# maxgillett/tinysplat

Measured on AMD Instinct MI355X. Metric: Gaussians*pixels/s fwd+bwd, higher is better.
Workload: dtype f32; 1 GPU; 1000000 random Gaussians, SH degree 3, 1920x1080, fwd+bwd (RGB), BASELINE configs[2]; max_per_tile=614, parallelism=single GPU, tile_lists=16x16 (gsplat's) (auto), gaussian_order=as generated (i.i.d.)

## Files before the change

tinysplat_amd/csrc/binning.hip:

```cpp
#include <hip/hip_runtime.h>

#include "../../include/tinysplat_hip.h"
#include "host_util.h"
#include "pack.h"
#include "row_spans.h"
#include "splat_math.h"

namespace {

constexpr int kThreads = 256;
constexpr int kScanItems = 4;
constexpr int kScanBlock = kThreads * kScanItems;

__device__ __forceinline__ int wave_inclusive_scan(int v) {
    const int lane = threadIdx.x & 63;
#pragma unroll
    for (int d = 1; d < 64; d <<= 1) {
        const int u = __shfl_up(v, d, 64);
        if (lane >= d) v += u;
    }
    return v;
}

template <int WAVES = 4>
// ... 989 lines not shown
    } else {
        walk([&](int t, int len, int i) {
            const int at = atomicAdd(&c.cursor[t >> kCoarseShift], len);
            for (int q = 0; q < len; ++q) dst[at + q] = i | (((t + q) & (kCoarseTiles - 1)) << kCoarseIdBits);
        });
    }
}

#ifndef TS_RUN_AHEAD
#define TS_RUN_AHEAD 20
#endif
constexpr int kRunItems = TS_RUN_AHEAD;
constexpr int kRunPass = kFineThreads * kRunItems;
#ifndef TS_RUNS_IN_FLIGHT
#define TS_RUNS_IN_FLIGHT 8
#endif
constexpr int kRunAhead = TS_RUNS_IN_FLIGHT;
__global__ __launch_bounds__(kFineThreads) void bin_scatter_fine_runs_kernel(
    int num_tiles, int groups, int chunks, const int* __restrict__ counts, const int* __restrict__ starts,
    int* __restrict__ tile_start, int* __restrict__ tile_bins, int* __restrict__ group_max,
    const int* __restrict__ scratch, int* __restrict__ bucket_ids) {
    extern __shared__ unsigned int buf[];
    const int my_count = (int)threadIdx.x < chunks ? counts[(size_t)threadIdx.x * groups + blockIdx.x] : 0;
    const int my_start = (int)threadIdx.x < chunks ? starts[(size_t)threadIdx.x * groups + blockIdx.x] : 0;
    const int begin = tile_start[min(num_tiles, (int)(blockIdx.x << kCoarseShift))];
    if (tile_start[num_tiles + 1] != 0) return;
    __shared__ FineGroup sh;
    __shared__ int roff[kBinMaxChunks + 1], rsrc[kBinMaxChunks];
    constexpr int kWaves = kFineThreads / 64;
    const int tid = threadIdx.x, lane = tid & 63, wave = tid >> 6;
    const int t0 = blockIdx.x << kCoarseShift, t1 = min(num_tiles, t0 + kCoarseTiles);
    if (tid < kCoarseTiles) {
        sh.hist[tid] = 0;
        sh.cursor[tid] = 0;
    }
    int total;
    {
        const int c = my_count;
        const int inc = block_inclusive_scan<kWaves>(c, &total);
        if (tid < chunks) {
            roff[tid] = inc - c;
            rsrc[tid] = my_start;
        }
        if (tid == 0) roff[chunks] = total;
    }
    __syncthreads();
    auto for_runs = [&](int c0, int m, auto op) {
#pragma unroll 1
        for (int b0 = wave; b0 < chunks; b0 += kWaves * kRunAhead) {
            int len[kRunAhead], src[kRunAhead], dst[kRunAhead];
            unsigned int v[kRunAhead];
#pragma unroll
            for (int u = 0; u < kRunAhead; ++u) {
                const int b = b0 + u * kWaves;
                len[u] = src[u] = dst[u] = 0;
                if (b < chunks) {
                    const int o = roff[b], c = roff[b + 1] - o;
                    const int lo = max(0, c0 - o) + lane;
                    len[u] = min(c, c0 + m - o) - lo;
                    src[u] = rsrc[b] + lo;
                    dst[u] = o - c0 + lo;
                }
            }
#pragma unroll
            for (int u = 0; u < kRunAhead; ++u)
                if (len[u] > 0) v[u] = (unsigned int)scratch[src[u]];
#pragma unroll
            for (int u = 0; u < kRunAhead; ++u)
                if (len[u] > 0) op(dst[u], v[u]);
#pragma unroll
            for (int u = 0; u < kRunAhead; ++u)
                for (int j = 64; j < len[u]; j += 64) op(dst[u] + j, (unsigned int)scratch[src[u] + j]);
        }
    };
    const GroupLists lists{t0, t1, begin, tile_start, tile_bins, group_max};
    const bool counted = total > kRunPass || total == 0;
    if (counted) {
        for_runs(0, total, [&](int, unsigned int w) { atomicAdd(&sh.hist[w >> kCoarseIdBits], 1); });
        publish_counted(sh, lists);
    }
    for (int c0 = 0; c0 < total; c0 += kRunPass) {
        const int m = min(kRunPass, total - c0);
        for_runs(c0, m, [&](int k, unsigned int w) { buf[k] = w; });
        __syncthreads();
        place_pass<kRunItems>(sh, buf, m, [&](int k) { return buf[k]; }, !counted, lists, bucket_ids);
    }
}

struct ListStats {
    const int* group_max;
    const int* guard;
    int* longest_out;
    int groups;
};
__device__ __forceinline__ void store_longest(const ListStats& st) {
    __shared__ int longest;
    if (threadIdx.x == 0) longest = 0;
    __syncthreads();
    int m = 0;
    for (int g = threadIdx.x; g < st.groups; g += kThreads) m = max(m, st.group_max[g]);
#pragma unroll
    for (int d = 32; d >= 1; d >>= 1) m = max(m, __shfl_xor(m, d, 64));
    if ((threadIdx.x & 63) == 0) atomicMax(&longest, m);
    __syncthreads();
    if (threadIdx.x == 0 && *st.guard == 0) *st.longest_out = longest;
}

constexpr int kSortCap = 4096;

#include "sort_network.h"

struct IdKeyArray {
    volatile int* ids;
    const float* depths;
};

__device__ __forceinline__ void cmpswap(IdKeyArray a, int i, int j) {
    const int x = a.ids[i], y = a.ids[j];
    if (make_key(a.depths, x) > make_key(a.depths, y)) { a.ids[i] = y; a.ids[j] = x; }
}

template <typename Ptr>
__device__ __forceinline__ void bitonic_network(Ptr a, int n) {
    int lg = 0;
    while ((1 << lg) < n) ++lg;
    const int half = (1 << lg) >> 1;
    for (int lk = 1; lk <= lg; ++lk) {
        const int k = 1 << lk, hk = k >> 1;
        for (int p = threadIdx.x; p < half; p += kThreads) {
            const int base = (p >> (lk - 1)) << lk, off = p & (hk - 1);
            const int i = base + off, j = base + k - 1 - off;
            if (j < n) cmpswap(a, i, j);
        }
        __syncthreads();
        for (int ld = lk - 2; ld >= 0; --ld) {
            const int d = 1 << ld;
            for (int p = threadIdx.x; p < half; p += kThreads) {
                const int i = ((p >> ld) << (ld + 1)) | (p & (d - 1)), j = i + d;
                if (j < n) cmpswap(a, i, j);
            }
            __syncthreads();
        }
    }
}

template <int E>
__device__ __forceinline__ void sort_tile_regs(const int* g, const float* __restrict__ depths,
                                               int* out, int n, unsigned long long* lds) {
    const int t = threadIdx.x;
    unsigned long long k[E];
#pragma unroll
    for (int e = 0; e < E; ++e) {
        const int i = t * E + e;
        k[e] = i < n ? make_key(depths, g[i]) : ~0ull;
    }
    __syncthreads();
    bitonic_regs<E, kThreads>(k, t, min(pow2_at_least(n), kThreads * E), lds);
#pragma unroll
    for (int e = 0; e < E; ++e) {
        const int i = t * E + e;
        if (i < n) out[i] = (int)(unsigned int)k[e];
    }
}

__device__ __forceinline__ void sort_bucket_block(const int* g, const float* __restrict__ depths,
                                                  int* out, int n, unsigned long long* lds) {
    if (n <= kThreads) sort_tile_regs<1>(g, depths, out, n, lds);
    else if (n <= 2 * kThreads) sort_tile_regs<2>(g, depths, out, n, lds);
    else if (n <= 4 * kThreads) sort_tile_regs<4>(g, depths, out, n, lds);
    else if (n <= 8 * kThreads) sort_tile_regs<8>(g, depths, out, n, lds);
    else sort_tile_regs<16>(g, depths, out, n, lds);
}

constexpr int kMaxSub = 512;
constexpr int kSubTarget = 96;
constexpr int kLargeLdsU64 = kSortCap + 2048;

__device__ __forceinline__ void sort_tile_sample(const int* __restrict__ g,
                                                 const float* __restrict__ depths,
                                                 int* __restrict__ out, int n,
                                                 unsigned long long* lds) {
    unsigned long long* scratch = lds;
    unsigned long long* smp = lds + kSortCap;
    int* start = reinterpret_cast<int*>(lds + kSortCap + 1024);
    int* cursor = start + (kMaxSub + 1);
    int* big = cursor + kMaxSub;
    __shared__ int nbig;
    const int t = threadIdx.x, lane = t & 63, wave = t >> 6;
    const int ns = n > 8192 ? 1024 : 256;
    int nb = n / kSubTarget;
    nb = nb < 2 ? 2 : (nb > kMaxSub ? kMaxSub : nb);

    if (ns == 1024) {
        unsigned long long k[4];
#pragma unroll
        for (int e = 0; e < 4; ++e)
            k[e] = make_key(depths, g[(int)(((long long)(t * 4 + e) * n) >> 10)]);
        bitonic_regs<4, kThreads>(k, t, 1024, scratch);
#pragma unroll
        for (int e = 0; e < 4; ++e) smp[t * 4 + e] = k[e];
    } else {
        unsigned long long k[1];
        k[0] = make_key(depths, g[(int)(((long long)t * n) >> 8)]);
        bitonic_regs<1, kThreads>(k, t, 256, scratch);
        smp[t] = k[0];
    }
    for (int b = t; b < nb; b += kThreads) cursor[b] = 0;
    if (t == 0) nbig = 0;
    __syncthreads();

    auto sub_of = [&](unsigned long long key) {
        int lo = 0, hi = nb - 1;
        while (lo < hi) {
            const int mid = (lo + hi) >> 1;
            if (smp[((mid + 1) * ns) / nb] <= key) lo = mid + 1; else hi = mid;
        }
        return lo;
    };
    for (int i = t; i < n; i += kThreads) atomicAdd(&cursor[sub_of(make_key(depths, g[i]))], 1);
    __syncthreads();
    {
        const int c0 = (2 * t < nb) ? cursor[2 * t] : 0, c1 = (2 * t + 1 < nb) ? cursor[2 * t + 1] : 0;
        int total;
        const int inc = block_inclusive_scan(c0 + c1, &total);
        const int ex = inc - (c0 + c1);
        if (2 * t < nb) start[2 * t] = ex;
        if (2 * t + 1 < nb) start[2 * t + 1] = ex + c0;
        if (t == 0) start[nb] = n;
    }
    __syncthreads();
    for (int b = t; b < nb; b += kThreads) cursor[b] = start[b];
    __syncthreads();
    for (int i = t; i < n; i += kThreads) {
        const int id = g[i];
        out[atomicAdd(&cursor[sub_of(make_key(depths, id))], 1)] = id;
    }
    __threadfence_block();
    __syncthreads();
    for (int b = wave; b < nb; b += kThreads / 64) {
        const int s0 = start[b], m = start[b + 1] - s0;
        if (m <= 1) continue;
        if (m <= 256) {
            unsigned long long k[4];
#pragma unroll
            for (int e = 0; e < 4; ++e) {
                const int i = lane * 4 + e;
                k[e] = i < m ? make_key(depths, out[s0 + i]) : ~0ull;
            }
            bitonic_regs<4, 64>(k, lane, min(pow2_at_least(m), 256), nullptr);
#pragma unroll
            for (int e = 0; e < 4; ++e) {
                const int i = lane * 4 + e;
                if (i < m) out[s0 + i] = (int)(unsigned int)k[e];
            }
        } else if (lane == 0) {
            big[atomicAdd(&nbig, 1)] = b;
        }
    }
    __syncthreads();
    const int nbg = nbig;
    for (int q = 0; q < nbg; ++q) {
        const int b = big[q];
        const int s0 = start[b], m = start[b + 1] - s0;
        __syncthreads();
        if (m <= kSortCap) {
            sort_bucket_block(out + s0, depths, out + s0, m, scratch);
        } else {
            IdKeyArray a{out + s0, depths};
            bitonic_network(a, m);
        }
        __syncthreads();
    }
}

__global__ __launch_bounds__(kThreads) void sort_tiles_small_kernel(
    int num_tiles, const int* __restrict__ tile_bins, const float* __restrict__ depths,
    const int* __restrict__ bucket_ids, int* __restrict__ ids_sorted, int* __restrict__ large_count,
    int* __restrict__ large_list, const ListStats stats) {
    if (stats.group_max && blockIdx.x == 0) store_longest(stats);
    const int lane = threadIdx.x & 63;
    const int tile = blockIdx.x * (kThreads / 64) + (threadIdx.x >> 6);
    if (tile >= num_tiles) return;
    const int2 range = reinterpret_cast<const int2*>(tile_bins)[tile];
    const int n = range.y - range.x;
    if (n <= 0) return;
    if (n > kWaveSortMax) {
        if (n > kSortCap && lane == 0) large_list[atomicAdd(large_count, 1)] = tile;
        return;
    }
    const int* g = bucket_ids + range.x;
    int* out = ids_sorted + range.x;
    if (n <= 64) sort_tile_wave<1>(g, depths, out, n, lane);
    else if (n <= 128) sort_tile_wave<2>(g, depths, out, n, lane);
    else if (n <= 256) sort_tile_wave<4>(g, depths, out, n, lane);
    else if (n <= 512) sort_tile_wave<8>(g, depths, out, n, lane);
    else sort_tile_wave<16>(g, depths, out, n, lane);
}

__global__ __launch_bounds__(kThreads) void sort_tiles_mid_kernel(
    const int* __restrict__ tile_bins, const float* __restrict__ depths,
    const int* __restrict__ bucket_ids, int* __restrict__ ids_sorted, int* __restrict__ large_count,
    int* __restrict__ large_list) {
    __shared__ unsigned long long lk[kSortCap / 2];
    const int2 range = reinterpret_cast<const int2*>(tile_bins)[blockIdx.x];
    const int n = range.y - range.x;
    if (n > kSortCap && large_count && threadIdx.x == 0) large_list[atomicAdd(large_count, 1)] = blockIdx.x;
    if (n <= kWaveSortMax || n > kSortCap) return;
    sort_bucket_block(bucket_ids + range.x, depths, ids_sorted + range.x, n, lk);
}

__global__ __launch_bounds__(kThreads) void sort_tiles_large_kernel(
    const int* __restrict__ tile_bins, const float* __restrict__ depths,
    const int* __restrict__ bucket_ids, int* __restrict__ ids_sorted,
    const int* __restrict__ large_count, const int* __restrict__ large_list) {
    __shared__ unsigned long long lds_large[kLargeLdsU64];
    const int count = *large_count;
    for (int q = blockIdx.x; q < count; q += gridDim.x) {
        const int2 range = reinterpret_cast<const int2*>(tile_bins)[large_list[q]];
        const int n = range.y - range.x;
        if (n <= kSortCap) continue;
        __syncthreads();
        sort_tile_sample(bucket_ids + range.x, depths, ids_sorted + range.x, n, lds_large);
    }
}

__global__ __launch_bounds__(kThreads) void sort_tiles_above_kernel(
    const int* __restrict__ tile_bins, const float* __restrict__ depths,
    const int* __restrict__ bucket_ids, int* __restrict__ ids_sorted, const ListStats stats) {
    __shared__ unsigned long long lds_u64[kLargeLdsU64 > kSortCap / 2 ? kLargeLdsU64 : kSortCap / 2];
    if (stats.group_max && blockIdx.x == 0) store_longest(stats);
    const int2 range = reinterpret_cast<const int2*>(tile_bins)[blockIdx.x];
    const int n = range.y - range.x;
    if (n <= kWaveSortMax) return;
    if (n <= kSortCap) sort_bucket_block(bucket_ids + range.x, depths, ids_sorted + range.x, n, lds_u64);
    else sort_tile_sample(bucket_ids + range.x, depths, ids_sorted + range.x, n, lds_u64);
}

__global__ __launch_bounds__(kThreads) void pack_splats_kernel(int n, const ts::PackArgs a,
                                                              const float* __restrict__ colors) {
    const int i = blockIdx.x * kThreads + threadIdx.x;
    if (i >= n) return;
    if (a.radii[i] <= 0) return;
    float c0, c1, c2, c3 = 0.0f;
    if (a.channels == 4 && a.depths == nullptr) {
        const float4 c = reinterpret_cast<const float4*>(colors)[i];
        c0 = c.x; c1 = c.y; c2 = c.z; c3 = c.w;
    } else {
        c0 = colors[3 * i]; c1 = colors[3 * i + 1]; c2 = colors[3 * i + 2];
        if (a.channels == 4) c3 = a.depths[i];
    }
    ts::pack_one(a, i, c0, c1, c2, c3);
}

template <typename... Params, typename... Args>
void launch_with_lds(void (*kernel)(Params...), dim3 grid, dim3 block, size_t lds, hipStream_t s, Args... args) {
    if (lds > 64 * 1024)
        (void)hipFuncSetAttribute(reinterpret_cast<const void*>(kernel), hipFuncAttributeMaxDynamicSharedMemorySize,
                                  (int)lds);
    hipLaunchKernelGGL(kernel, grid, block, lds, s, args...);
}

}

extern "C" {

int32_t ts_num_tiles(const ts_camera* cam) {
    if (!cam) return 0;
    const int tbx = cam->wide_tiles ? (cam->tile_bounds_x + 1) / 2 : cam->tile_bounds_x;
    return cam->tile_rows * tbx;
}

int64_t ts_scan_ws_ints(int32_t n) {
    return n <= 0 ? 1 : (int64_t)((n + kScanBlock - 1) / kScanBlock);
}

int ts_scan_tiles(int32_t n, const int32_t* num_tiles_hit, int32_t* cum_tiles_hit,
                  int32_t* scan_ws, int32_t* total_out, void* stream) {
    if (n < 0) return TS_E_BADARG;
    if (n == 0) return 0;
    if (!num_tiles_hit || !cum_tiles_hit || !scan_ws) return TS_E_BADARG;
    hipStream_t s = (hipStream_t)stream;
    const int nb = (n + kScanBlock - 1) / kScanBlock;
    hipLaunchKernelGGL(scan_local_kernel, dim3(nb), dim3(kThreads), 0, s, n, num_tiles_hit,
                       cum_tiles_hit, scan_ws, total_out);
    if (nb > 1)
        hipLaunchKernelGGL(scan_add_kernel, dim3(nb), dim3(kThreads), 0, s, n, cum_tiles_hit, scan_ws,
                           total_out);
    return launch_status();
}

int64_t ts_bin_ws_ints(int32_t n, int32_t num_tiles) { return bin_geometry(n, num_tiles).spare + 1; }

int ts_bin_count(int32_t n, const float* xys, const int32_t* radii, const float* splats,
                 const ts_camera* cam, int32_t* bin_ws, void* stream) {
    if (n < 0 || !cam || !bin_ws) return TS_E_BADARG;
    const int nt = ts_num_tiles(cam);
    if (nt <= 0) return 0;
    if (n > 0 && (!xys || !radii)) return TS_E_BADARG;
    const BinGeometry g = bin_geometry(n, nt);
    const int window = bin_window_tiles(n, nt);
// ... 261 lines not shown
```

tinysplat_amd/csrc/raster.hip:

```cpp
#include <hip/hip_runtime.h>

#include <type_traits>

#include "../../include/tinysplat_hip.h"
#include "host_util.h"
#include "raster_survivors.h"
#include "splat_math.h"

namespace {
#include "sort_network.h"

#ifndef TS_FWD_MIN_WAVES_RGB
#define TS_FWD_MIN_WAVES_RGB 5
#endif
#ifndef TS_FWD_MIN_WAVES_RGBD
#define TS_FWD_MIN_WAVES_RGBD 5
#endif
#ifndef TS_BWD_MIN_WAVES_16
#define TS_BWD_MIN_WAVES_16 5
#endif

#ifndef TS_ABLATE
#define TS_ABLATE 0
#endif
// ... 298 lines not shown
        "v_fma_f32 %2, -%1, %5, %5\n\t"
        "v_sub_f32_e32 %3, %5, %2\n\t"
        "v_cmp_nge_f32_e32 vcc, %16, %2\n\t"
        "v_cndmask_b32_e32 %4, 0, %3, vcc\n\t"
        "v_fmac_f32_e32 %6, %11, %4\n\t"
        "v_fmac_f32_e32 %7, %12, %4\n\t"
        "v_cndmask_b32_e64 %5, -|%5|, %2, vcc\n\t"
        "v_fmac_f32_e32 %8, %13, %4\n\t"
        "v_cmp_lt_f32_e32 vcc, 0, %4\n\t"
        "v_cndmask_b32_e32 %9, %9, %14, vcc"
        : "=&v"(a), "=&v"(ae), "=&v"(nT), "=&v"(d), "=&v"(vis), "+v"(T), "+v"(a0), "+v"(a1), "+v"(a2), "+v"(fidx)
        : "v"(sgl), "v"(c0), "v"(c1), "v"(c2), "v"(idx), "s"(ts::kAlphaMin), "s"(ts::kTEps)
        : "vcc");
    return vis;
}
__device__ __forceinline__ float fwd_update(float ae, float& T, int& fidx, int idx, float& a0, float& a1, float& a2,
                                            float c0, float c1, float c2) {
    float nT, d, vis;
    asm("v_fma_f32 %0, -%8, %3, %3\n\t"
        "v_sub_f32_e32 %1, %3, %0\n\t"
        "v_cmp_nge_f32_e32 vcc, %13, %0\n\t"
        "v_cndmask_b32_e32 %2, 0, %1, vcc\n\t"
        "v_fmac_f32_e32 %4, %9, %2\n\t"
        "v_fmac_f32_e32 %5, %10, %2\n\t"
        "v_cndmask_b32_e64 %3, -|%3|, %0, vcc\n\t"
        "v_fmac_f32_e32 %6, %11, %2\n\t"
        "v_cmp_lt_f32_e32 vcc, 0, %2\n\t"
        "v_cndmask_b32_e32 %7, %7, %12, vcc"
        : "=&v"(nT), "=&v"(d), "=&v"(vis), "+v"(T), "+v"(a0), "+v"(a1), "+v"(a2), "+v"(fidx)
        : "v"(ae), "v"(c0), "v"(c1), "v"(c2), "v"(idx), "s"(ts::kTEps)
        : "vcc");
    return vis;
}

template <int CH, bool GENERAL, class Loc>
__device__ __forceinline__ void fwd_chunk(const float4* __restrict__ lds, int cnt, const float (&fpx)[NBC],
                                          const float (&fpy)[2], float (&T)[NB], int (&fidx)[NB],
                                          float (&acc)[NB][CH], Loc& loc TS_SEG_PARAM) {
#pragma clang fp contract(off)
    constexpr bool LOC = Loc::on;
    TS_WORK(0, cnt);
    for (int j = 0; j < (TS_ABLATE == 3 ? 0 : cnt); ++j) {
        TS_SEG_T0(tseg_a);
        const float4 r0 = lds[3 * j], r1 = lds[3 * j + 1], r2 = lds[3 * j + 2];
        const int bm = __builtin_amdgcn_readfirstlane(__float_as_int(r2.w));
        const int idx = __float_as_int(r2.z);
        const float neg_lo = -r1.y;
        float col[CH];
        col[0] = r1.z; col[1] = r1.w; col[2] = r2.x;
        if (CH == 4) col[CH - 1] = r2.y;
#if TS_TIMELINE
        asm volatile("s_waitcnt lgkmcnt(0)" ::: "memory");
#endif
        TS_SEG_ADD(ts_seg_, 1, tseg_a);
        TS_SEG_T0(tseg_b);
        TS_WORK(1, __popc(bm & ((1 << NB) - 1)));
#pragma unroll
        for (int k = 0; k < NB; ++k) {
            if (!(bm & (1 << k))) continue;
            if (TS_ABLATE == 5) { asm volatile("" ::: "memory"); continue; }
            TS_STAT(1, 1);
            const float sgl = sigma_l2(r0.z, r0.w, r1.x, neg_lo, r0.x - fpx[k % NBC], r0.y - fpy[k / NBC]);
            if (TS_ABLATE == 8) {
                float dup = sigma_l2(r0.z, r0.w, r1.x, neg_lo, r0.y - fpx[k % NBC], r0.x - fpy[k / NBC]);
                dup = __builtin_amdgcn_exp2f(-dup);
                asm volatile("" ::"v"(dup));
            }
            float vis;
            if (!GENERAL) {
                vis = fwd_alpha_update(sgl, T[k], fidx[k], idx, acc[k][0], acc[k][1], acc[k][2], col[0], col[1], col[2]);
            } else {
                float ae = fwd_alpha(sgl);
                ae = fminf(ts::kAlphaMax, ae);
                ae = sgl >= neg_lo ? ae : 0.0f;
                vis = fwd_update(ae, T[k], fidx[k], idx, acc[k][0], acc[k][1], acc[k][2], col[0], col[1], col[2]);
            }
            if (CH == 4) acc[k][CH - 1] = __builtin_fmaf(col[CH - 1], vis, acc[k][CH - 1]);
            if (LOC) loc.add(k, col, vis);
        }
        TS_SEG_ADD(ts_seg_, 2, tseg_b);
    }
}

#define TS_CAM_COOP16(cam) (((cam).hints >> 16) & 15)
static_assert(kWaves == 4, "a cooperative workgroup is one wave per 8x8 block of a 16x16 tile");
#ifndef TS_COOP_AHEAD
#define TS_COOP_AHEAD 4
#endif
constexpr int kCoopAhead = TS_COOP_AHEAD;
constexpr int kHintCoopAll = 1 << 21;
struct FwdPlan {
    int per_xcd;
    int coop, coop_lo;
    bool descending;
    __host__ __device__ int grid() const { return 8 * (per_xcd + (kWaves - 1) * coop); }
};
__host__ __device__ __forceinline__ FwdPlan fwd_plan(int num_tiles, int hints, bool segs, bool coop_ok) {
    FwdPlan p;
    const int groups = (num_tiles + kWaves - 1) / kWaves;
    p.per_xcd = (groups + 7) >> 3;
    const int w16 = (hints >> 12) & 15, c16 = (hints >> 16) & 15;
    const CutTiles m = cut_tiles(num_tiles, hints);
    if (coop_ok && (hints & kHintCoopAll) && !segs) {
        p.coop = p.per_xcd;
        p.coop_lo = 0;
        p.descending = false;
        return p;
    }
    if (segs && coop_ok && (hints & kHintCoopAll)) {
        p.coop = (m.band - m.whole) / kWaves;
        p.coop_lo = m.whole / kWaves;
        p.descending = false;
        return p;
    }
    p.coop = coop_ok ? (p.per_xcd * c16) / 16 : 0;
    if (segs) p.coop = w16 > 0 ? min(p.coop, m.whole / kWaves) : 0;
    p.coop_lo = 0;
    p.descending = (segs && w16 > 0) || p.coop > 0;
    return p;
}

template <int CH, bool GENERAL, bool LOC>
__device__ __forceinline__ void fwd_body1(const float4 r0, const float4 r1, const float4 r2, float fpx, float fpy,
                                          float& T, int& fidx, float (&acc)[CH], float (&loc)[CH]) {
#pragma clang fp contract(off)
    const int idx = __float_as_int(r2.z);
    const float neg_lo = -r1.y;
    float col[CH];
    col[0] = r1.z; col[1] = r1.w; col[2] = r2.x;
    if (CH == 4) col[CH - 1] = r2.y;
    const float sgl = sigma_l2(r0.z, r0.w, r1.x, neg_lo, r0.x - fpx, r0.y - fpy);
    float vis;
    if (!GENERAL) {
        vis = fwd_alpha_update(sgl, T, fidx, idx, acc[0], acc[1], acc[2], col[0], col[1], col[2]);
    } else {
        float ae = fwd_alpha(sgl);
        ae = fminf(ts::kAlphaMax, ae);
        ae = sgl >= neg_lo ? ae : 0.0f;
        vis = fwd_update(ae, T, fidx, idx, acc[0], acc[1], acc[2], col[0], col[1], col[2]);
    }
    if (CH == 4) acc[CH - 1] = __builtin_fmaf(col[CH - 1], vis, acc[CH - 1]);
    if (LOC) {
#pragma unroll
        for (int c = 0; c < CH; ++c) loc[c] = __builtin_fmaf(col[c], vis, loc[c]);
    }
}

template <int E>
__device__ __forceinline__ void coop_sort_run(const int* __restrict__ g, const float* __restrict__ depths, int n_run,
                                              int lane, unsigned long long (&k)[E]) {
#pragma unroll
    for (int e = 0; e < E; ++e) {
        const int i = e * 64 + lane;
        k[e] = i < n_run ? make_key(depths, g[i]) : ~0ull;
    }
    bitonic_regs<E, 64>(k, lane, E == 1 ? min(pow2_at_least(max(n_run, 1)), 64) : 64 * E, nullptr);
}
template <int E>
__device__ __forceinline__ void coop_sort_tile(const int* __restrict__ g, const float* __restrict__ depths,
                                               int* __restrict__ out, int* ids_l, int n, int wave, int lane,
                                               unsigned long long* keys) {
    const int q = (n + 3) >> 2;
    const int n_own = max(0, min(q, n - wave * q));
    unsigned long long k[E];
    coop_sort_run<E>(g + wave * q, depths, n_own, lane, k);
#pragma unroll
    for (int e = 0; e < E; ++e) keys[wave * 256 + lane * E + e] = k[e];
    TS_LDS_BARRIER();
    int lo[E][3], len[3];
#pragma unroll
    for (int dv = 0; dv < 3; ++dv) len[dv] = max(0, min(q, n - ((wave + dv + 1) & 3) * q));
#pragma unroll
    for (int e = 0; e < E; ++e)
#pragma unroll
        for (int dv = 0; dv < 3; ++dv) lo[e][dv] = 0;
#pragma unroll
    for (int step = 64 * E; step >= 1; step >>= 1) {
#pragma unroll
        for (int e = 0; e < E; ++e) {
#pragma unroll
            for (int dv = 0; dv < 3; ++dv) {
                const unsigned long long* run = keys + ((wave + dv + 1) & 3) * 256;
                const int p = lo[e][dv] + step;
                if (p <= len[dv] && run[p - 1] < k[e]) lo[e][dv] = p;
            }
        }
    }
#pragma unroll
    for (int e = 0; e < E; ++e) {
        const int p = lane * E + e;
        if (p < n_own) {
            const int rank = p + lo[e][0] + lo[e][1] + lo[e][2];
            out[rank] = (int)(unsigned int)k[e];
            ids_l[rank] = (int)(unsigned int)k[e];
        }
    }
}

template <int CH, bool SORT, bool SEGS, bool SURV>
__device__ __forceinline__ void coop_fwd_tile(
    const ts_camera& cam, int tile, int num_tiles, const int* __restrict__ tile_bins, const int* __restrict__ ids_sorted,
    const int* __restrict__ bucket_ids, const float* __restrict__ depths, int* ids_rw,
    const float4* __restrict__ splats, const float* __restrict__ background, float* __restrict__ out_img,
    float* __restrict__ out_depth, float* __restrict__ final_Ts, int* __restrict__ final_index, int clamp_rgb,
    unsigned char* __restrict__ clamp_mask, float4* rec, float4* rect_sh, int* cnt_sh, int* alive_sh, int clock_unit,
    int* sv_id, int* sv_meta, int* sv_cnt) {
    const int wave = threadIdx.x >> 6, lane = threadIdx.x & 63;
    const int tbx = cam.tile_bounds_x;
    const int tx = tile % tbx, ty = tile / tbx + cam.tile_row0;
    const int px = tx * 16 + 8 * (wave & 1) + (lane & 7), py = ty * 16 + 8 * (wave >> 1) + (lane >> 3);
    const float fpx = (float)px + ts::kPixOff, fpy = (float)py + ts::kPixOff;
    const float BX0 = (float)(tx * 16 + 8 * (wave & 1)) + ts::kPixOff, BY0 = (float)(ty * 16 + 8 * (wave >> 1)) + ts::kPixOff;
    const int W = cam.img_width, H = cam.img_height;
    const bool inside = px < W && py < H;
    float T = inside ? 1.0f : -1.0f, acc[CH];
    int fidx = 0;
#pragma unroll
    for (int c = 0; c < CH; ++c) acc[c] = 0.0f;
    const int2 range = reinterpret_cast<const int2*>(tile_bins)[tile];
    const int n = range.y - range.x;
    TS_WAVE_CLOCK(0, clock_unit + wave, n);
    (void)clock_unit;

    const int S_seg = max(1, min(TS_CAM_SEGS(cam), kSegMax));
    int ck_block = -1;
    if (SEGS && final_Ts != nullptr && S_seg > 1 && n >= kSegMinList) ck_block = cut_tiles(num_tiles, cam.hints).block_of(tile);
    const bool seg_on = SEGS && ck_block >= 0;
    float* ckp = nullptr;
    if (seg_on) ckp = final_Ts + ckpt_offset(seg_plane_stride(cam)) + ckpt_record<CH>(ck_block, S_seg, 1);
    int next_ck = seg_on ? range.x + seg_bound(n, S_seg, 1) : 0x7fffffff;
    int ck = 1;
    float loc[CH];
#pragma unroll
    for (int c = 0; c < CH; ++c) loc[c] = 0.0f;
    auto store_ck = [&](int number) {
        ckpt_store<CH>(ckp + (number - 1) * ((1 + CH) * 256), wave, lane, __builtin_fabsf(T), loc);
#pragma unroll
        for (int c = 0; c < CH; ++c) loc[c] = 0.0f;
    };

    auto publish = [&]() {
        const unsigned long long m = __ballot(T > 0.0f);
        int xmin = 0, xmax = 0, ymin = 0, ymax = 0;
        const bool any = mask_rect(m, xmin, xmax, ymin, ymax);
        if (lane == 0) {
            alive_sh[wave] = any ? 1 : 0;
            if (any) rect_sh[wave] = make_float4(BX0 + (float)xmin, BX0 + (float)xmax, BY0 + (float)ymin, BY0 + (float)ymax);
        }
    };
    publish();

    int idr[4] = {0, 0, 0, 0};
    bool from_lds = false;
    TS_SEG_T0(tseg_s);
    if (SORT && TS_ABLATE == 6 && n <= kWaveSortMax) {
        for (int i = threadIdx.x; i < n; i += 256) ids_rw[range.x + i] = bucket_ids[range.x + i];
        __builtin_amdgcn_fence(__ATOMIC_SEQ_CST, "workgroup");
        __syncthreads();
    } else
    if (SORT && n > 0 && n <= kWaveSortMax) {
        const int* g = bucket_ids + range.x;
        int* out = ids_rw + range.x;
        if (n <= 128) {
            if (wave == 0) {
                if (n <= 64) sort_tile_wave<1>(g, depths, out, n, lane);
                else sort_tile_wave<2>(g, depths, out, n, lane);
            }
        } else {
            unsigned long long* keys = reinterpret_cast<unsigned long long*>(rec);
            int* ids_l = reinterpret_cast<int*>(rec) + 2048;
            if (n <= 256) coop_sort_tile<1>(g, depths, out, ids_l, n, wave, lane, keys);
            else if (n <= 512) coop_sort_tile<2>(g, depths, out, ids_l, n, wave, lane, keys);
            else coop_sort_tile<4>(g, depths, out, ids_l, n, wave, lane, keys);
        }
        if (n <= 128) {
            __builtin_amdgcn_fence(__ATOMIC_SEQ_CST, "workgroup");
            __syncthreads();
        } else {
            TS_LDS_BARRIER();
            const int* ids_l = reinterpret_cast<const int*>(rec) + 2048;
#pragma unroll
            for (int r = 0; r < 4; ++r) {
                const int i = 256 * r + 64 * wave + lane;
                if (i < n) idr[r] = ids_l[i];
            }
            from_lds = true;
        }
    }
    TS_SEG_ADD(ts_wave_clock_.seg, 3, tseg_s);
    const int* ids = SORT ? ids_rw : ids_sorted;

    const float4 zero4 = make_float4(0.f, 0.f, 0.f, 0.f);
    float4 n0 = zero4, n1 = zero4, n2 = zero4;
    int id_next = 0;
    int g_n = 0;
    {
        const int i0 = range.x + 64 * wave + lane;
        if (i0 < range.y) {
            const int g = from_lds ? idr[0] : ids[i0];
            n0 = splats[3 * (size_t)g]; n1 = splats[3 * (size_t)g + 1]; n2 = splats[3 * (size_t)g + 2];
            g_n = g;
        }
        if (i0 + 256 < range.y) id_next = from_lds ? idr[1] : ids[i0 + 256];
    }
    int nsv = 0;
    int round = 0;
    for (int base = range.x; base < range.y; base += 256) {
// ... 1266 lines not shown
```

tinysplat_amd/csrc/sort_network.h:

```cpp
#pragma once

__device__ __forceinline__ unsigned long long make_key(const float* __restrict__ depths, int id) {
    return ((unsigned long long)__float_as_uint(depths[id]) << 32) | (unsigned int)id;
}


template <int M>
__device__ __forceinline__ unsigned int lane_xor_dpp(unsigned int x) {
    static_assert(M == 1 || M == 2 || M == 4 || M == 8, "DPP reaches lane ^ 1, 2, 4, 8");
    const int v = (int)x;
    if constexpr (M == 1) return (unsigned int)__builtin_amdgcn_update_dpp(0, v, 0xB1, 0xF, 0xF, true);
    if constexpr (M == 2) return (unsigned int)__builtin_amdgcn_update_dpp(0, v, 0x4E, 0xF, 0xF, true);
    if constexpr (M == 8) return (unsigned int)__builtin_amdgcn_update_dpp(0, v, 0x128, 0xF, 0xF, true);
    if constexpr (M == 4) {
        const int r = __builtin_amdgcn_update_dpp(0, v, 0x141, 0xF, 0xF, true);
        return (unsigned int)__builtin_amdgcn_update_dpp(0, r, 0x1B, 0xF, 0xF, true);
    }
    return x;
}

template <int E, int M>
__device__ __forceinline__ void exchange_stage_dpp(unsigned long long (&k)[E], bool keep_min) {
#pragma unroll
    for (int e = 0; e < E; ++e) {
        const unsigned long long o = ((unsigned long long)lane_xor_dpp<M>((unsigned int)(k[e] >> 32)) << 32) |
                                     lane_xor_dpp<M>((unsigned int)k[e]);
        k[e] = ((o < k[e]) == keep_min) ? o : k[e];
    }
}

template <int E, int GROUP>
__device__ __forceinline__ void bitonic_regs(unsigned long long (&k)[E], int t, int npad,
                                             unsigned long long* lds) {
    constexpr bool kDpp = GROUP > 64;
    const int lane = t & 63;
    for (int kk = 2; kk <= npad; kk <<= 1) {
        for (int j = kk >> 1; j >= E && j >= 1; j >>= 1) {
            const bool asc = ((t * E) & kk) == 0;
            if (GROUP > 64 && j >= 64 * E) {
                constexpr int H = E >= 2 ? E / 2 : 1;
                const bool keep_min = (((t * E) & j) == 0) == asc;
                const int partner = t ^ (j / E);
#pragma unroll
                for (int r = 0; r < E / H; ++r) {
#pragma unroll
                    for (int e = 0; e < H; ++e) lds[e * GROUP + t] = k[r * H + e];
                    __syncthreads();
#pragma unroll
                    for (int e = 0; e < H; ++e) {
                        const unsigned long long o = lds[e * GROUP + partner];
                        k[r * H + e] = ((o < k[r * H + e]) == keep_min) ? o : k[r * H + e];
                    }
                    __syncthreads();
                }
            } else {
                const int m = j / E;
                const bool keep_min = ((lane & m) == 0) == asc;
                switch (kDpp ? m : 0) {
                    case 1: exchange_stage_dpp<E, 1>(k, keep_min); break;
                    case 2: exchange_stage_dpp<E, 2>(k, keep_min); break;
                    case 4: exchange_stage_dpp<E, 4>(k, keep_min); break;
                    case 8: exchange_stage_dpp<E, 8>(k, keep_min); break;
                    default:
#pragma unroll
                        for (int e = 0; e < E; ++e) {
                            const unsigned long long o = __shfl_xor(k[e], m, 64);
                            k[e] = ((o < k[e]) == keep_min) ? o : k[e];
                        }
                }
            }
        }
#pragma unroll
        for (int jj = E >> 1; jj >= 1; jj >>= 1) {
            if (jj < kk) {
#pragma unroll
                for (int e = 0; e < E; ++e) {
                    if ((e & jj) == 0) {
                        const bool asc = (((t * E + e) & kk) == 0);
                        const unsigned long long x = k[e], y = k[e | jj];
                        const bool sw = (x > y) == asc;
                        k[e] = sw ? y : x;
                        k[e | jj] = sw ? x : y;
                    }
                }
            }
        }
    }
}

__device__ __forceinline__ int pow2_at_least(int n) {
    int p = 2;
    while (p < n) p <<= 1;
    return p;
}


#ifndef TS_WAVE_SORT_MAX
#define TS_WAVE_SORT_MAX 1024
#endif
constexpr int kWaveSortMax = TS_WAVE_SORT_MAX;
template <int E>
__device__ __forceinline__ void sort_tile_wave(const int* __restrict__ g,
                                               const float* __restrict__ depths,
                                               int* __restrict__ out, int n, int lane) {
    unsigned long long k[E];
#pragma unroll
    for (int e = 0; e < E; ++e) {
        const int i = e * 64 + lane;
        k[e] = i < n ? make_key(depths, g[i]) : ~0ull;
    }
    bitonic_regs<E, 64>(k, lane, min(pow2_at_least(n), 64 * E), nullptr);
#pragma unroll
    for (int e = 0; e < E; ++e) {
        const int i = lane * E + e;
        if (i < n) out[i] = (int)(unsigned int)k[e];
    }
}
```

Baseline: 2095000 billion Gaussians*pixels/s.

## Use f64 min/max instructions for bitonic compare-exchange with sign-flip direction trick

```diff
diff --git a/tinysplat_amd/csrc/binning.hip b/tinysplat_amd/csrc/binning.hip
--- a/tinysplat_amd/csrc/binning.hip
+++ b/tinysplat_amd/csrc/binning.hip
@@ -1165,7 +1165,7 @@
 #pragma unroll
     for (int e = 0; e < E; ++e) {
         const int i = t * E + e;
-        k[e] = i < n ? make_key(depths, g[i]) : ~0ull;
+        k[e] = i < n ? make_key(depths, g[i]) : kKeyPad;
     }
     __syncthreads();
     bitonic_regs<E, kThreads>(k, t, min(pow2_at_least(n), kThreads * E), lds);
@@ -1258,7 +1258,7 @@
 #pragma unroll
             for (int e = 0; e < 4; ++e) {
                 const int i = lane * 4 + e;
-                k[e] = i < m ? make_key(depths, out[s0 + i]) : ~0ull;
+                k[e] = i < m ? make_key(depths, out[s0 + i]) : kKeyPad;
             }
             bitonic_regs<4, 64>(k, lane, min(pow2_at_least(m), 256), nullptr);
 #pragma unroll
diff --git a/tinysplat_amd/csrc/raster.hip b/tinysplat_amd/csrc/raster.hip
--- a/tinysplat_amd/csrc/raster.hip
+++ b/tinysplat_amd/csrc/raster.hip
@@ -474,7 +474,7 @@
 #pragma unroll
     for (int e = 0; e < E; ++e) {
         const int i = e * 64 + lane;
-        k[e] = i < n_run ? make_key(depths, g[i]) : ~0ull;
+        k[e] = i < n_run ? make_key(depths, g[i]) : kKeyPad;
     }
     bitonic_regs<E, 64>(k, lane, E == 1 ? min(pow2_at_least(max(n_run, 1)), 64) : 64 * E, nullptr);
 }
diff --git a/tinysplat_amd/csrc/sort_network.h b/tinysplat_amd/csrc/sort_network.h
--- a/tinysplat_amd/csrc/sort_network.h
+++ b/tinysplat_amd/csrc/sort_network.h
@@ -1,7 +1,21 @@
 #pragma once
 
+constexpr unsigned long long kKeyPad = 0x7FF0000000000000ull;
 __device__ __forceinline__ unsigned long long make_key(const float* __restrict__ depths, int id) {
     return ((unsigned long long)__float_as_uint(depths[id]) << 32) | (unsigned int)id;
+}
+
+__device__ __forceinline__ void cmpx_f64(unsigned long long& x, unsigned long long& y) {
+    unsigned long long lo, hi;
+    asm("v_min_f64 %0, %1, %2" : "=v"(lo) : "v"(x), "v"(y));
+    asm("v_max_f64 %0, %1, %2" : "=v"(hi) : "v"(x), "v"(y));
+    x = lo;
+    y = hi;
+}
+__device__ __forceinline__ unsigned long long min_neg_f64(unsigned long long k, unsigned long long o) {
+    unsigned long long r;
+    asm("v_min_f64 %0, %1, -%2" : "=v"(r) : "v"(k), "v"(o));
+    return r;
 }
 
 
@@ -33,10 +47,35 @@
 __device__ __forceinline__ void bitonic_regs(unsigned long long (&k)[E], int t, int npad,
                                              unsigned long long* lds) {
     constexpr bool kDpp = GROUP > 64;
+    constexpr bool kMinNeg = GROUP == 64;
     const int lane = t & 63;
-    for (int kk = 2; kk <= npad; kk <<= 1) {
+#pragma unroll
+    for (int kk = 2; kk < E; kk <<= 1) {
+        if (kk <= npad) {
+#pragma unroll
+            for (int jj = kk >> 1; jj >= 1; jj >>= 1) {
+#pragma unroll
+                for (int e = 0; e < E; ++e) {
+                    if ((e & jj) == 0) {
+                        if ((e & kk) == 0) cmpx_f64(k[e], k[e | jj]);
+                        else cmpx_f64(k[e | jj], k[e]);
+                    }
+                }
+            }
+        }
+    }
+    unsigned int sign = 0;
+    auto to_state = [&](bool negated) {
+        const unsigned int want = negated ? 0x80000000u : 0u;
+        const unsigned long long toggle = (unsigned long long)(want ^ sign) << 32;
+        sign = want;
+#pragma unroll
+        for (int e = 0; e < E; ++e) k[e] ^= toggle;
+    };
+    for (int kk = E > 2 ? E : 2; kk <= npad; kk <<= 1) {
+        const bool asc = ((t * E) & kk) == 0;
+        if (E > 1 && !kMinNeg) to_state(!asc);
         for (int j = kk >> 1; j >= E && j >= 1; j >>= 1) {
-            const bool asc = ((t * E) & kk) == 0;
             if (GROUP > 64 && j >= 64 * E) {
                 constexpr int H = E >= 2 ? E / 2 : 1;
                 const bool keep_min = (((t * E) & j) == 0) == asc;
@@ -56,6 +95,7 @@
             } else {
                 const int m = j / E;
                 const bool keep_min = ((lane & m) == 0) == asc;
+                if (kMinNeg) to_state(!keep_min);
                 switch (kDpp ? m : 0) {
                     case 1: exchange_stage_dpp<E, 1>(k, keep_min); break;
                     case 2: exchange_stage_dpp<E, 2>(k, keep_min); break;
@@ -65,27 +105,24 @@
 #pragma unroll
                         for (int e = 0; e < E; ++e) {
                             const unsigned long long o = __shfl_xor(k[e], m, 64);
-                            k[e] = ((o < k[e]) == keep_min) ? o : k[e];
+                            if (kMinNeg) k[e] = min_neg_f64(k[e], o);
+                            else k[e] = ((o < k[e]) == keep_min) ? o : k[e];
                         }
                 }
             }
         }
+        if (E > 1) {
+            if (kMinNeg) to_state(!asc);
 #pragma unroll
-        for (int jj = E >> 1; jj >= 1; jj >>= 1) {
-            if (jj < kk) {
+            for (int jj = E >> 1; jj >= 1; jj >>= 1) {
 #pragma unroll
                 for (int e = 0; e < E; ++e) {
-                    if ((e & jj) == 0) {
-                        const bool asc = (((t * E + e) & kk) == 0);
-                        const unsigned long long x = k[e], y = k[e | jj];
-                        const bool sw = (x > y) == asc;
-                        k[e] = sw ? y : x;
-                        k[e | jj] = sw ? x : y;
-                    }
+                    if ((e & jj) == 0) cmpx_f64(k[e], k[e | jj]);
                 }
             }
         }
     }
+    to_state(false);
 }
 
 __device__ __forceinline__ int pow2_at_least(int n) {
@@ -107,7 +144,7 @@
 #pragma unroll
     for (int e = 0; e < E; ++e) {
         const int i = e * 64 + lane;
-        k[e] = i < n ? make_key(depths, g[i]) : ~0ull;
+        k[e] = i < n ? make_key(depths, g[i]) : kKeyPad;
     }
     bitonic_regs<E, 64>(k, lane, min(pow2_at_least(n), 64 * E), nullptr);
 #pragma unroll
```

Measured after the change: 2115000 billion Gaussians*pixels/s (median of 6 runs). About the same (+1.0%).
